# sangyun884/HR-VITON

Measured on AMD Instinct MI355X. Metric: 1024x768 try-on images/sec (train_generator.py step: tocg+glue, G fwd/bwd, D fwd/bwd x2, VGG, Adam), higher is better.
Workload: dtype bf16; 1 GPU; BASELINE configs[3] (SURVEY 8d config #4, headline): train_generator.py 1024x768, 4 img/GPU, --fp16 (bf16 MFMA operands, fp32 accumulate), SPADE ng...; global_batch=4, height=1024, width=768, parallelism=dp1-allreduce, persistent_grid_cus=256, dist_backend=none (single process), world_size=1, rccl_ranks=0

## Files before the change

hr-viton_amd/csrc/conv_f32.hip:

```cpp
#include <stdarg.h>
#include <stdlib.h>
#include <string.h>

#include <vector>

#include "conv_params.h"

namespace hrv {

template <int TM, int TN, int WM, int WN, int VAR, bool BF, int RB = 64>
__device__ __forceinline__ void conv_mfma_tile(const ConvParams& p, const int bid) {
  static_assert(WM * WN == 4 || WM * WN == 8, "4 or 8 MMA waves per block");
  constexpr int NT = 64 * WM * WN;
  constexpr bool SPEC = (VAR & 32) != 0;
  static_assert(RB == 64 || RB == 128, "K-tile row = 64 or 128 bytes");
  constexpr int ES = BF ? 2 : 4;
  constexpr int EPG = 16 / ES;
  constexpr int GPR = RB / 16;
  constexpr int BKE = GPR * EPG;
  constexpr bool GLDS = (VAR & 4) != 0;
  static_assert(!GLDS || (BF && RB == 128), "the LDS-DMA variant exists for the bf16 engine with 128-byte rows");
  constexpr bool SF = (VAR & 8) != 0;
  static_assert(!SF || (BF && !GLDS), "fp32-source variant: bf16 MFMA, register-staged");
  constexpr int LS = GLDS ? RB / 4 : RB / 4 + 4;
  constexpr int BK = RB / 4;
  constexpr int KQ = RB / 32;
  constexpr int RPP = NT / GPR;
  constexpr int BM = 32 * TM * WM;
  constexpr int BN = 32 * TN * WN;
  constexpr int AR = BM / RPP;
  constexpr int BR = (BN * GPR + NT - 1) / NT;
  constexpr bool SWAP = (VAR & 1) != 0;
  constexpr bool PIPE = (VAR & 2) != 0;
  constexpr int ST = (VAR & 16) ? 3 : 2;
  static_assert(ST == 2 || GLDS, "the 3-stage pipeline exists for the LDS-DMA variant");
  static_assert(!SPEC || ST == 3, "wave specialisation rides on the 3-stage LDS-DMA pipeline");
// ... 545 lines not shown
#undef HRV_ADVANCE_ITER
#undef HRV_STORE_TILE
#undef HRV_READ_FRAGS
#undef HRV_MMA1
#undef HRV_MMA_FRAGS

  if (p.splitk > 1) {
    float* wsp = p.ws + (size_t)ks * p.M * p.CoutPad;
#pragma unroll
    for (int j = 0; j < TN; ++j)
#pragma unroll
      for (int i = 0; i < TM; ++i) {
        if (SWAP) {
          const int pidx = row2pix((wm * TM + i) * 32 + l31);
#pragma unroll
          for (int g = 0; g < 4; ++g) {
            const int c0 = n0 + (wn * TN + j) * 32 + 8 * g + 4 * lh;
            if (pidx < p.M) {
              f32x4 v;
#pragma unroll
              for (int e = 0; e < 4; ++e) v[e] = acc[i][j][4 * g + e];
              *reinterpret_cast<f32x4*>(wsp + (size_t)pidx * p.CoutPad + c0) = v;
            }
          }
        } else {
          const int c = n0 + (wn * TN + j) * 32 + l31;
#pragma unroll
          for (int e = 0; e < 16; ++e) {
            const int pidx = row2pix((wm * TM + i) * 32 + 4 * lh + (e & 3) + 8 * (e >> 2));
            if (pidx < p.M) wsp[(size_t)pidx * p.CoutPad + c] = acc[i][j][e];
          }
        }
      }
    return;
  }
  if (!SWAP) {
#pragma unroll
    for (int j = 0; j < TN; ++j) {
      const int c = n0 + (wn * TN + j) * 32 + l31;
      const bool c_ok = c < p.Cout;
      const float sc = (c_ok && p.scale) ? p.scale[c] : 1.f;
      const float sh = (c_ok && p.shift) ? p.shift[c] : 0.f;
#pragma unroll
      for (int i = 0; i < TM; ++i) {
        const int prow0 = (wm * TM + i) * 32 + 4 * lh;
#pragma unroll
        for (int e = 0; e < 16; ++e) {
          const int pidx = row2pix(prow0 + (e & 3) + 8 * (e >> 2));
          if (c_ok && pidx < p.M) {
            float v = acc[i][j][e] * sc + sh;
            const size_t opix = out_pixel(p, pidx);
            if (p.res) v = res_combine(v, ld1rt<BF>(p.res, opix * p.res_cs + p.res_co + c, p.res_f32), p.res_mode, p.slope);
            v = apply_act(v, p.act, p.slope);
            if (!p.out_up) {
              st1rt<BF>(p.out, opix * p.out_cs + p.out_co + c, v, p.out_f32);
            } else {
              const int n = pidx / (p.Ho * p.Wo), rem = pidx - n * (p.Ho * p.Wo);
              const int h = rem / p.Wo, w = rem - h * p.Wo;
              const size_t o = (((size_t)n * 2 * p.Ho + 2 * h) * 2 * p.Wo + 2 * w) * p.out_cs + p.out_co + c;
              st1rt<BF>(p.out, o, v, p.out_f32); st1rt<BF>(p.out, o + p.out_cs, v, p.out_f32);
              st1rt<BF>(p.out, o + (size_t)2 * p.Wo * p.out_cs, v, p.out_f32); st1rt<BF>(p.out, o + (size_t)2 * p.Wo * p.out_cs + p.out_cs, v, p.out_f32);
            }
          }
        }
      }
    }
  } else {
// ... 372 lines not shown

struct TileCfg {
  int TM, TN, WM, WN;
  int RB;
};
static const TileCfg kCfgs[] = {
    {2, 2, 2, 2, 64},
    {1, 3, 4, 1, 64},
    {2, 3, 4, 1, 64},
    {2, 1, 4, 1, 64},
    {2, 2, 4, 1, 64},
    {1, 1, 4, 1, 64},
    {1, 2, 4, 1, 64},
    {4, 2, 2, 2, 64},
    {2, 2, 2, 2, 128},
    {1, 2, 4, 1, 128},
    {4, 2, 2, 2, 128},
    {2, 4, 2, 2, 128},
    {2, 2, 4, 2, 128},
    {2, 2, 4, 2, 128},
    {4, 2, 2, 2, 128},
    {2, 2, 2, 2, 128},
    {2, 2, 4, 2, 128},
    {2, 2, 2, 2, 128},
    {1, 2, 4, 1, 128},
    {2, 2, 4, 1, 128},
};
constexpr int kNumCfgs = sizeof(kCfgs) / sizeof(kCfgs[0]);

static int cfg_bm(int c) { return 32 * kCfgs[c].TM * kCfgs[c].WM; }
static int cfg_bn(int c) { return 32 * kCfgs[c].TN * kCfgs[c].WN; }
static int cfg_rb(int c) { return kCfgs[c].RB; }

static int pick_splitk(int nblk, int KT, bool allowed) {
  if (!allowed || nblk >= 768 || KT < 16) return 1;
  int s = (1024 + nblk - 1) / nblk;
  if (s > 32) s = 32;
  if (s > KT / 8) s = KT / 8;
  return s < 2 ? 1 : s;
}

static int fill_params(const hrv_conv2d_t* d, ConvParams& p, bool need_packed, bool bf = false) {
  const bool srcf = bf && d && ((d->mixed_flags >> 3) & 1);
  const int cm = (bf && !srcf) ? 8 : 4;
  HRV_REQUIRE(d != nullptr, "conv2d: null descriptor");
  const int rb = (need_packed && d->tile_cfg >= 0 && d->tile_cfg < kNumCfgs) ? cfg_rb(d->tile_cfg) : 64;
  HRV_REQUIRE(bf || rb == 64, "conv2d: tile_cfg=%d (128-byte K-tile rows) exists on the bf16 engine only", d->tile_cfg);
  const int bke = rb / (bf ? 2 : 4);
  HRV_REQUIRE(d->nsrc >= 1 && d->nsrc <= HRV_MAX_SRC, "conv2d: nsrc=%d out of range", d->nsrc);
  HRV_REQUIRE(d->N > 0 && d->H > 0 && d->W > 0 && d->Ho > 0 && d->Wo > 0, "conv2d: bad extent");
  HRV_REQUIRE(d->KH > 0 && d->KW > 0 && d->stride > 0 && d->pad >= 0, "conv2d: bad kernel geometry");
  const int padw = d->pad_w_plus1 > 0 ? d->pad_w_plus1 - 1 : d->pad;
  HRV_REQUIRE(d->free_extent ||
                  (d->Ho == (d->H + 2 * d->pad - d->KH) / d->stride + 1 && d->Wo == (d->W + 2 * padw - d->KW) / d->stride + 1),
              "conv2d: Ho/Wo (%d,%d) inconsistent with H,W,k,stride,pad", d->Ho, d->Wo);
  HRV_REQUIRE(d->out_step == 0 || (d->out_step == 2 && d->out_up_shift == 0 && !d->spade && d->out_off_h >= 0 &&
                                   d->out_off_w >= 0 && 2 * (d->Ho - 1) + d->out_off_h < d->out_H &&
                                   2 * (d->Wo - 1) + d->out_off_w < d->out_W),
              "conv2d: out_step/out_off/out_H/out_W inconsistent");
  HRV_REQUIRE(d->res_mode == 0 || d->res_mode == 1, "conv2d: res_mode");
  HRV_REQUIRE(d->Cout > 0 && d->out != nullptr, "conv2d: bad output");
  HRV_REQUIRE((int64_t)d->N * d->Ho * d->Wo < (int64_t)1 << 31, "conv2d: too many output pixels");
  memset(&p, 0, sizeof(p));
  p.bf16 = bf ? 1 : 0;
  p.out_f32 = bf ? (d->mixed_flags & 1) : 1;
  p.res_f32 = bf ? ((d->mixed_flags >> 1) & 1) : 1;
  p.sx_f32 = bf ? ((d->mixed_flags >> 2) & 1) : 1;
  p.src_f32 = srcf ? 1 : 0;
  HRV_REQUIRE(!srcf || rb == 128, "conv2d: fp32-source bf16 mode needs a 128-byte-row tile (cfg 8/9)");
  p.nsrc = d->nsrc;
  int chunks_total = 0;
  bool dma_ok = bf && rb == 128 && !srcf;
// ... 47 lines not shown
  if (d->spade) {
    const hrv_spade_epi_t& e = *d->spade;
    HRV_REQUIRE(need_packed, "conv2d: the SPADE epilogue exists on the MFMA engine only");
    HRV_REQUIRE(e.x && e.mean && e.rstd && d->shift, "conv2d/spade: null pointer");
    HRV_REQUIRE(e.C > 0 && e.C % 4 == 0 && e.x_cstride % 4 == 0 && e.x_coff % 4 == 0 && e.x_coff + e.C <= e.x_cstride,
                "conv2d/spade: channels must be multiples of 4 and in range");
    HRV_REQUIRE(d->Cout == (e.C + 31) / 32 * 64, "conv2d/spade: Cout must be 2*ceil32(C) = %d", (e.C + 31) / 32 * 64);
    HRV_REQUIRE(d->stride == 1 && d->Ho == d->H && d->Wo == d->W, "conv2d/spade: 'same' stride-1 geometry only");
    HRV_REQUIRE((e.noise_z == nullptr) == (e.noise_scale == nullptr), "conv2d/spade: noise_z/noise_scale go together");
    HRV_REQUIRE(d->out_cstride % 4 == 0 && d->out_coff % 4 == 0 && d->out_cstride >= d->out_coff + e.C,
                "conv2d/spade: out slice");
    HRV_REQUIRE((((uintptr_t)e.x | (uintptr_t)e.mean | (uintptr_t)e.rstd | (uintptr_t)e.noise_scale |
                  (uintptr_t)d->shift | (uintptr_t)d->out) & 15) == 0, "conv2d/spade: 16-byte alignment");
    p.epi = 1; p.sx = e.x; p.sx_cs = e.x_cstride; p.sx_co = e.x_coff; p.sC = e.C;
    p.smean = e.mean; p.srstd = e.rstd; p.sz = e.noise_z; p.sns = e.noise_scale; p.sg1p = e.g1p_out;
    p.res = nullptr; p.scale = nullptr;
  } else {
    HRV_REQUIRE(d->out_cstride >= d->out_coff + d->Cout, "conv2d: out slice out of range");
  }
  HRV_REQUIRE(d->residual == nullptr || d->res_cstride >= d->res_coff + d->Cout, "conv2d: residual slice out of range");
  if (need_packed) {
    HRV_REQUIRE(d->tile_cfg >= 0 && d->tile_cfg < kNumCfgs, "conv2d: tile_cfg=%d invalid", d->tile_cfg);
    HRV_REQUIRE(d->w_packed != nullptr && ((uintptr_t)d->w_packed & 15) == 0, "conv2d: w_packed null/unaligned");
    const int bm = cfg_bm(d->tile_cfg), bn = cfg_bn(d->tile_cfg);
    p.wp = (const float*)d->w_packed;
    p.n_tiles = (d->Cout + bn - 1) / bn;
    p.CoutPad = p.n_tiles * bn;
    {
      const int64_t wb = (int64_t)p.KT * p.CoutPad * rb;
      p.w_bytes = (dma_ok && wb < (int64_t)0xFFFFFFF0) ? (unsigned)wb : 0u;
    }
    p.m_tiles = (p.M + bm - 1) / bm;
    p.splitk = 1;
    const char* ev = hrv::env("HRV_CONV_SPLITK");
    int want = pick_splitk(p.m_tiles * p.n_tiles, p.KT, d->spade == nullptr);
    if (ev) want = atoi(ev) > 0 ? atoi(ev) : 1;
    if (d->spade) want = 1;
    if (want > p.KT) want = p.KT;
    if (want > 1) {
      const int64_t need = (int64_t)want * p.M * p.CoutPad * (int64_t)sizeof(float);
      if (d->workspace && d->workspace_bytes >= need && (((uintptr_t)d->workspace) & 15) == 0) {
        p.splitk = want;
        p.ws = (float*)d->workspace;
      }
    }
  } else {
    p.splitk = 1;
  }
  return HRV_OK;
}

constexpr int kDefaultVariant = 1;

template <int TM, int TN, int WM, int WN, int RB = 64>
static int launch_cfg(const ConvParams& p, hipStream_t st) {
  const int nblk = p.m_tiles * p.n_tiles * p.splitk;
  const char* ev = hrv::env("HRV_CONV_VARIANT");
  int var = ev ? atoi(ev) : kDefaultVariant;
  const int oesz = p.out_f32 ? 4 : 2, resz = p.res_f32 ? 4 : 2;
  const bool vec_ok = (p.Cout & 3) == 0 && ((p.out_cs | p.out_co) & 3) == 0 && (!p.res || ((p.res_cs | p.res_co) & 3) == 0) &&
                      (((uintptr_t)p.scale | (uintptr_t)p.shift) & 15) == 0 && (((uintptr_t)p.out) & (4 * oesz - 1)) == 0 &&
                      (((uintptr_t)p.res) & (4 * resz - 1)) == 0;
  if (p.epi == 1) {
    if (TN % 2 != 0) { set_error("conv2d/spade: tile_cfg must have an even TN (cfg 0, 4, 6 or 7)"); return HRV_ERR_ARG; }
    var |= 1;
  } else if (!vec_ok) {
    var &= ~1;
  }
  if (p.bf16) {
    if constexpr (RB == 128 && (32 * TN * WN * 8) % 256 == 0) {
      const char* eg = hrv::env("HRV_CONV_GLDS");
      const bool want = eg ? atoi(eg) != 0 : (32 * TN * WN == 64 || TM * TN >= 8);
      const bool glds = want && p.w_bytes != 0;
      if (p.src_f32) {
        if (var & 1) hipLaunchKernelGGL((conv_mfma_kernel<TM, TN, WM, WN, 9, true, RB>), dim3(nblk), dim3(64 * WM * WN), 0, st, p);
        else hipLaunchKernelGGL((conv_mfma_kernel<TM, TN, WM, WN, 8, true, RB>), dim3(nblk), dim3(64 * WM * WN), 0, st, p);
      } else if (glds) {
        if (var & 1) hipLaunchKernelGGL((conv_mfma_kernel<TM, TN, WM, WN, 5, true, RB>), dim3(nblk), dim3(64 * WM * WN), 0, st, p);
        else hipLaunchKernelGGL((conv_mfma_kernel<TM, TN, WM, WN, 4, true, RB>), dim3(nblk), dim3(64 * WM * WN), 0, st, p);
      } else {
        if (var & 1) hipLaunchKernelGGL((conv_mfma_kernel<TM, TN, WM, WN, 1, true, RB>), dim3(nblk), dim3(64 * WM * WN), 0, st, p);
        else hipLaunchKernelGGL((conv_mfma_kernel<TM, TN, WM, WN, 0, true, RB>), dim3(nblk), dim3(64 * WM * WN), 0, st, p);
      }
    } else {
      if (var & 1) hipLaunchKernelGGL((conv_mfma_kernel<TM, TN, WM, WN, 1, true, RB>), dim3(nblk), dim3(64 * WM * WN), 0, st, p);
      else hipLaunchKernelGGL((conv_mfma_kernel<TM, TN, WM, WN, 0, true, RB>), dim3(nblk), dim3(64 * WM * WN), 0, st, p);
    }
  } else if constexpr (RB != 64) {
    set_error("conv2d: 128-byte K-tile rows exist on the bf16 engine only");
    return HRV_ERR_ARG;
  } else {
    switch (var) {
      case 0: hipLaunchKernelGGL((conv_mfma_kernel<TM, TN, WM, WN, 0, false>), dim3(nblk), dim3(64 * WM * WN), 0, st, p); break;
      case 1: hipLaunchKernelGGL((conv_mfma_kernel<TM, TN, WM, WN, 1, false>), dim3(nblk), dim3(64 * WM * WN), 0, st, p); break;
      case 2: hipLaunchKernelGGL((conv_mfma_kernel<TM, TN, WM, WN, 2, false>), dim3(nblk), dim3(64 * WM * WN), 0, st, p); break;
      case 3: hipLaunchKernelGGL((conv_mfma_kernel<TM, TN, WM, WN, 3, false>), dim3(nblk), dim3(64 * WM * WN), 0, st, p); break;
      default: set_error("conv2d: HRV_CONV_VARIANT=%d invalid", var); return HRV_ERR_ARG;
    }
  }
  int rc = check_launch("conv_mfma_kernel");
  if (rc || p.splitk <= 1) return rc;
  const size_t total = (size_t)p.M * ((p.Cout + 3) / 4);
  const size_t gsz = (total + 255) / 256;
  const dim3 g((unsigned)(gsz > 4096 ? 4096 : gsz));
  if (p.bf16) hipLaunchKernelGGL(splitk_reduce_kernel<true>, g, dim3(256), 0, st, p);
  else hipLaunchKernelGGL(splitk_reduce_kernel<false>, g, dim3(256), 0, st, p);
  return check_launch("splitk_reduce_kernel");
}

template <int TM, int TN, int WM, int WN, bool ST3, bool SPECW = false>
static int launch_cfg8w(const ConvParams& p, hipStream_t st) {
  const int nblk = p.m_tiles * p.n_tiles * p.splitk;
  const int oesz = p.out_f32 ? 4 : 2, resz = p.res_f32 ? 4 : 2;
  const bool vec_ok = (p.Cout & 3) == 0 && ((p.out_cs | p.out_co) & 3) == 0 && (!p.res || ((p.res_cs | p.res_co) & 3) == 0) &&
                      (((uintptr_t)p.scale | (uintptr_t)p.shift) & 15) == 0 && (((uintptr_t)p.out) & (4 * oesz - 1)) == 0 &&
                      (((uintptr_t)p.res) & (4 * resz - 1)) == 0;
  if (!p.bf16 || p.src_f32 || p.w_bytes == 0) {
    set_error("conv2d: tile_cfg 12/13 (eight-wave LDS-DMA) needs bf16-stored sources within the 32-bit buffer range");
    return HRV_ERR_ARG;
  }
  constexpr int V = 4 | (ST3 ? 16 : 0) | (SPECW ? 32 : 0);
  constexpr int NTB = 64 * WM * WN * (SPECW ? 2 : 1);
  if (vec_ok || p.epi == 1)
    hipLaunchKernelGGL((conv_mfma_kernel<TM, TN, WM, WN, V | 1, true, 128>), dim3(nblk), dim3(NTB), 0, st, p);
  else
    hipLaunchKernelGGL((conv_mfma_kernel<TM, TN, WM, WN, V, true, 128>), dim3(nblk), dim3(NTB), 0, st, p);
  int rc = check_launch("conv_mfma_kernel");
  if (rc || p.splitk <= 1) return rc;
  const size_t total = (size_t)p.M * ((p.Cout + 3) / 4);
  const size_t gsz = (total + 255) / 256;
  const dim3 g((unsigned)(gsz > 4096 ? 4096 : gsz));
  hipLaunchKernelGGL(splitk_reduce_kernel<true>, g, dim3(256), 0, st, p);
  return check_launch("splitk_reduce_kernel");
}

static bool patch_eligible(const ConvParams& p) {
  return p.bf16 && !p.src_f32 && p.nsrc == 1 && p.KH == 3 && p.KW == 3 && p.stride == 1 && p.pad == 1 && p.pad_w == 1 &&
         p.Ho == p.H && p.Wo == p.W && p.src[0].up_shift == 0 && p.src[0].C % 128 == 0 && p.src[0].bytes != 0 &&
         p.w_bytes != 0 && p.out_step != 2;
}

template <int TMP, int TNP, int WMP, int WNP, int STV>
static int launch_patch(const ConvParams& p0, hipStream_t st, int n0_base = 0, int n_cols_tiles = 0) {
  constexpr int BNP = 32 * TNP * WNP;
  if (!patch_eligible(p0) || (n_cols_tiles == 0 && p0.CoutPad % BNP != 0) || n0_base + n_cols_tiles * BNP > p0.CoutPad) {
    set_error("conv2d: tile_cfg 16-18 (patch mode) needs a 3x3 stride-1 'same' convolution over one bf16-stored source with "
              "C %% 128 == 0");
    return HRV_ERR_ARG;
  }
  ConvParams p = p0;
  p.splitk = 1;
  constexpr int THP = TMP * WMP * 32 / 16;
  p.m_tiles = p.N * ((p.H + THP - 1) / THP) * ((p.W + 15) / 16);
  p.n_tiles = n_cols_tiles > 0 ? n_cols_tiles : p.CoutPad / BNP;
  p.n0_base = n0_base;
  const int nblk = p.m_tiles * p.n_tiles;
  const int oesz = p.out_f32 ? 4 : 2, resz = p.res_f32 ? 4 : 2;
  const bool vec_ok = (p.Cout & 3) == 0 && ((p.out_cs | p.out_co) & 3) == 0 && (!p.res || ((p.res_cs | p.res_co) & 3) == 0) &&
                      (((uintptr_t)p.scale | (uintptr_t)p.shift) & 15) == 0 && (((uintptr_t)p.out) & (4 * oesz - 1)) == 0 &&
                      (((uintptr_t)p.res) & (4 * resz - 1)) == 0;
  constexpr int V = 4 | STV | 64;
  const int n_cu = persistent_cus();
  p.tlog = diag_tlog(p.m_tiles);
  constexpr int PATCH_LDS = ((TMP * WMP * 32 / 16 + 2) * 18 * 64 + ((STV & 16) ? 3 : 2) * BNP * 32) * 4;
  const int per_cu = PATCH_LDS <= 80 * 1024 ? 2 : 1;
  const char* ep = hrv::env("HRV_PATCH_PERSIST");
  int grid = (ep && ep[0] == '0') ? nblk : n_cu * per_cu;
  if (grid > nblk) grid = nblk;
  if (vec_ok || p.epi == 1)
    hipLaunchKernelGGL((conv_mfma_kernel<TMP, TNP, WMP, WNP, V | 1, true, 128>), dim3(grid), dim3(64 * WMP * WNP), 0, st, p);
  else
    hipLaunchKernelGGL((conv_mfma_kernel<TMP, TNP, WMP, WNP, V, true, 128>), dim3(grid), dim3(64 * WMP * WNP), 0, st, p);
  return check_launch("conv_mfma_kernel[patch]");
}

static int launch_any(int tile_cfg, const ConvParams& p, hipStream_t st) {
  switch (tile_cfg) {
    case 0: return launch_cfg<2, 2, 2, 2>(p, st);
    case 1: return launch_cfg<1, 3, 4, 1>(p, st);
    case 2: return launch_cfg<2, 3, 4, 1>(p, st);
    case 3: return launch_cfg<2, 1, 4, 1>(p, st);
    case 4: return launch_cfg<2, 2, 4, 1>(p, st);
    case 5: return launch_cfg<1, 1, 4, 1>(p, st);
    case 6: return launch_cfg<1, 2, 4, 1>(p, st);
    case 7: return launch_cfg<4, 2, 2, 2>(p, st);
    case 8: return launch_cfg<2, 2, 2, 2, 128>(p, st);
    case 9: return launch_cfg<1, 2, 4, 1, 128>(p, st);
    case 10: return launch_cfg<4, 2, 2, 2, 128>(p, st);
    case 11: return launch_cfg<2, 4, 2, 2, 128>(p, st);
    case 12: return launch_cfg8w<2, 2, 4, 2, false>(p, st);
    case 13: return launch_cfg8w<2, 2, 4, 2, true>(p, st);
    case 14: return launch_cfg8w<4, 2, 2, 2, true, true>(p, st);
    case 15: return launch_cfg8w<2, 2, 2, 2, true, true>(p, st);
    case 16: return launch_patch<2, 2, 4, 2, 16>(p, st);
    case 17: return launch_patch<2, 2, 2, 2, 0>(p, st);
    case 18: {
      const char* e3 = hrv::env("HRV_CONV_PATCH_ST3");
      if (e3 && e3[0] == '0') return launch_patch<1, 2, 4, 1, 0>(p, st);
      const char* es = hrv::env("HRV_CONV_PATCH_SPLIT");
      const int c64 = p.CoutPad / 64;
      if (c64 >= 3 && !(es && es[0] == '0')) {
        const int rc = launch_patch<2, 2, 2, 2, 0>(p, st, 0, c64 / 2);
        if (rc) return rc;
        return launch_patch<1, 2, 4, 1, 16>(p, st, (c64 / 2) * 128, c64 - 2 * (c64 / 2));
      }
      return launch_patch<1, 2, 4, 1, 16>(p, st);
    }
    case 19: return launch_patchw(p, st);
  }
  set_error("conv2d: tile_cfg=%d invalid", tile_cfg);
  return HRV_ERR_ARG;
}

}

using namespace hrv;

extern "C" int hrv_conv2d_tile_bn(int32_t c) { return (c >= 0 && c < kNumCfgs) ? cfg_bn(c) : -1; }
extern "C" int hrv_conv2d_tile_bm(int32_t c) { return (c >= 0 && c < kNumCfgs) ? cfg_bm(c) : -1; }
extern "C" int hrv_conv2d_tile_row_bytes(int32_t c) { return (c >= 0 && c < kNumCfgs) ? cfg_rb(c) : -1; }
// ... 33 lines not shown
  HRV_REQUIRE(tile_cfg >= 0 && tile_cfg < kNumCfgs && cfg_rb(tile_cfg) == 64, "pack_weight: bad tile_cfg %d", tile_cfg);
  HRV_REQUIRE(nsrc >= 1 && nsrc <= HRV_MAX_SRC, "pack_weight: bad nsrc");
  constexpr int BK = HOST_BK;
  const int bn = cfg_bn(tile_cfg);
  const int64_t cpad = (int64_t)((Cout + bn - 1) / bn) * bn;
  int cin_real = 0, chunks_total = 0;
  for (int i = 0; i < nsrc; ++i) {
    HRV_REQUIRE(srcC_real[i] > 0 && srcC_real[i] <= srcC[i] && srcC[i] % 4 == 0, "pack_weight: bad channel counts");
    cin_real += srcC_real[i];
    chunks_total += (srcC[i] + BK - 1) / BK;
  }
  const int64_t total = (int64_t)KH * KW * chunks_total * cpad * BK;
  memset(out, 0, sizeof(float) * total);
  for (int kh = 0; kh < KH; ++kh)
    for (int kw = 0; kw < KW; ++kw) {
      int chunk0 = 0, cbase = 0;
      for (int s = 0; s < nsrc; ++s) {
        const int chunks = (srcC[s] + BK - 1) / BK;
        for (int c = 0; c < srcC_real[s]; ++c) {
          const int64_t kt = (int64_t)(kh * KW + kw) * chunks_total + chunk0 + c / BK;
          float* dst = out + (kt * cpad) * BK + (c % BK);
          const float* srcw = w + ((int64_t)(cbase + c) * KH + kh) * KW + kw;
          const int64_t ostride = (int64_t)cin_real * KH * KW;
          for (int co = 0; co < Cout; ++co) dst[(int64_t)co * BK] = srcw[co * ostride];
        }
        chunk0 += chunks;
        cbase += srcC_real[s];
      }
    }
  return HRV_OK;
}

extern "C" int64_t hrv_conv2d_workspace_bytes(const hrv_conv2d_t* d) {
  if (!d || d->tile_cfg < 0 || d->tile_cfg >= kNumCfgs || d->spade) return 0;
  const int bm = cfg_bm(d->tile_cfg), bn = cfg_bn(d->tile_cfg);
  const int64_t M = (int64_t)d->N * d->Ho * d->Wo;
  const int n_tiles = (d->Cout + bn - 1) / bn;
  const int m_tiles = (int)((M + bm - 1) / bm);
  int chunks = 0;
  for (int i = 0; i < d->nsrc && i < HRV_MAX_SRC; ++i) chunks += (d->src[i].C + HOST_BK - 1) / HOST_BK;
  const int KT = d->KH * d->KW * chunks;
  const char* ev = hrv::env("HRV_CONV_SPLITK");
  int s = pick_splitk(m_tiles * n_tiles, KT, true);
  if (ev) s = atoi(ev) > 0 ? atoi(ev) : 1;
  if (s > KT) s = KT;
  return s > 1 ? (int64_t)s * M * n_tiles * bn * (int64_t)sizeof(float) : 0;
}

static int conv2d_one(const hrv_conv2d_t* d, hipStream_t stream, bool bf) {
  ConvParams p;
  int rc = fill_params(d, p, true, bf);
  if (rc) return rc;
  return launch_any(d->tile_cfg, p, stream);
}

static int conv2d_any(const hrv_conv2d_t* d, hipStream_t stream, bool bf) {
  HRV_REQUIRE(d != nullptr, "conv2d: null descriptor");
  HRV_REQUIRE(d->nsrc >= 1 && d->nsrc <= HRV_MAX_SRC && d->N > 0 && d->H > 0 && d->W > 0, "conv2d: bad geometry");
  int64_t per_img = 0;
  for (int i = 0; i < d->nsrc; ++i) {
    const hrv_src_t& s = d->src[i];
    const int sr = s.up_shift > 0 ? s.up_shift : 0, sl = s.up_shift < 0 ? -s.up_shift : 0;
    const int64_t e = (int64_t)((d->H >> sr) << sl) * ((d->W >> sr) << sl) * s.cstride;
    per_img = e > per_img ? e : per_img;
  }
  const int64_t out_px = (int64_t)d->Ho * d->Wo;
  const bool srcf0 = bf && (d->mixed_flags & 8);
  const int64_t lim = (int64_t)0xFFFFFFF0 / ((bf && !srcf0) ? 2 : 4);
  int64_t cap = d->N;
  if (const char* e = hrv::env("HRV_CONV_MAX_BATCH")) {
    const long long v = atoll(e);
    if (v > 0 && v < cap) cap = v;
  }
  const bool fits = cap == d->N && d->N * per_img < lim && d->N * out_px < ((int64_t)1 << 31);
  const bool plain_fwd = d->out_step <= 1 && d->free_extent == 0 && d->res_mode == 0;
  if (fits || !plain_fwd || per_img <= 0 || out_px <= 0) return conv2d_one(d, stream, bf);
  int64_t nb = (lim - 1) / per_img;
  const int64_t nb2 = (((int64_t)1 << 31) - 1) / out_px;
  nb = nb < nb2 ? nb : nb2;
// ... 118 lines not shown
```

hr-viton_amd/csrc/conv_params.h:

```cpp
#pragma once
#include "hrv_common.h"

namespace hrv {

typedef float f32x16 __attribute__((ext_vector_type(16)));
typedef float f32x4 __attribute__((ext_vector_type(4)));

constexpr int HOST_BK = 16;

struct SrcDev {
  const float* ptr;
  int C, cstride, coff, up_shift, pre_act, chunks;
  unsigned bytes;
};

struct ConvParams {
  SrcDev src[HRV_MAX_SRC];
  int nsrc;
  int N, H, W, Ho, Wo, KH, KW, stride, pad;
  int M;
  int Cout, CoutPad;
  int chunks_total;
  int KT;
  int m_tiles, n_tiles;
  int n0_base;
  const float* wp;
  const float* scale;
  const float* shift;
  const float* res;
  int res_cs, res_co;
  int act;
  float slope;
  float pre_slope;
  float* out;
  int out_cs, out_co;
  int splitk;
  float* ws;
  int pad_w;
  int out_up;
  int out_step, out_oh, out_ow, out_H, out_W;
  int bf16;
  int out_f32, res_f32, sx_f32;
  int src_f32;
  int res_mode;
  unsigned w_bytes;
  int epi;
  const float* sx;
  int sx_cs, sx_co, sC;
  const float* smean;
  const float* srstd;
  const float* sz;
  const float* sns;
  float* sg1p;
  unsigned long long* tlog;
};

__device__ __forceinline__ size_t out_pixel(const ConvParams& p, int pidx) {
  if (p.out_step != 2) return (size_t)pidx;
  const int n = pidx / (p.Ho * p.Wo), rem = pidx - n * (p.Ho * p.Wo);
  const int h = rem / p.Wo, w = rem - h * p.Wo;
  return ((size_t)n * p.out_H + 2 * h + p.out_oh) * p.out_W + 2 * w + p.out_ow;
}

__device__ __forceinline__ float res_combine(float v, float r, int mode, float slope) {
  return mode == 0 ? v + r : v * (r > 0.f ? 1.f : slope);
}

typedef __bf16 bf16x8 __attribute__((ext_vector_type(8)));
typedef unsigned short u16x4 __attribute__((ext_vector_type(4)));

// ... 92 lines not shown
```

hr-viton_amd/ops.py:

```python
from __future__ import annotations

import ctypes as C
import os
from dataclasses import dataclass
from typing import Optional, Sequence, Tuple, Union

import weakref

import torch

from . import _lib
from ._lib import ACT_LRELU, ACT_NONE, ACT_RELU, ACT_TANH, HrvError


WEIGHTS_EPOCH = [0]
LOAD_EPOCH = [0]


def weights_epoch(tensors) -> int:
    return sum(getattr(t, "_hrv_epoch", 0) for t in tensors)


def _ceil4(c: int) -> int:
    return (c + 3) // 4 * 4
# ... 148 lines not shown
    _Prof.enabled = False
    torch.cuda.synchronize()
    out = [((k, n, fl, by, s.elapsed_time(e), kn) if kernels else (k, n, fl, by, s.elapsed_time(e)))
           for (k, n, fl, by, kn, s, e) in _Prof.records]
    _Prof.records = []
    return out


class _Timed:
    def __init__(self, kind, name, flops, nbytes, kernel=None):
        self.args = (kind, name, flops, nbytes, kernel or kind)

    def __enter__(self):
        if _Prof.enabled:
            self.s = torch.cuda.Event(enable_timing=True)
            self.e = torch.cuda.Event(enable_timing=True)
            self.s.record()
        return self

    def __exit__(self, *a):
        if _Prof.enabled:
            self.e.record()
            _Prof.records.append((*self.args, self.s, self.e))
        return False


_WS = {}
GRAPH_WATCH = weakref.WeakSet()


WS_PER_STREAM = [False]


def _workspace(device, nbytes: int) -> torch.Tensor:
    key = (str(device), torch.cuda.current_stream(device).cuda_stream if WS_PER_STREAM[0] else 0)
    t = _WS.get(key)
    if t is None or t.numel() * 4 < nbytes:
        t = torch.empty((nbytes + 3) // 4, dtype=torch.float32, device=device)
        _WS[key] = t
    return t


SrcSpec = Union[Act, Tuple[Act, int, int]]


class ConvLayer:

    def __init__(self, weight: torch.Tensor, src_real: Sequence[int], device, scale: Optional[torch.Tensor] = None,
                 shift: Optional[torch.Tensor] = None, stride: int = 1, pad: int = 1, act: int = ACT_NONE,
                 slope: float = 0.2, name: str = "conv", bf16: bool = False, out_f32: bool = False,
                 mma_bf16: bool = False):
        assert not (bf16 and mma_bf16)
        self.bf16 = bf16
        self.mixed = mma_bf16
        self.out_f32 = out_f32 or not bf16
        w = weight.detach().to("cpu", torch.float32).contiguous()
        self.Cout, cin, self.KH, self.KW = w.shape
        assert sum(src_real) == cin, (name, src_real, cin)
        assert 1 <= len(src_real) <= _lib.HRV_MAX_SRC
        self.w_cpu = w
        self.src_real = list(src_real)
        self.src_pad = [_cpad(c, bf16) for c in src_real]
        self.device = device
        self.stride, self.pad, self.act, self.slope, self.name = stride, pad, act, slope, name
        self.scale = None if scale is None else scale.detach().to(device, torch.float32).contiguous()
        self.shift = None if shift is None else shift.detach().to(device, torch.float32).contiguous()
        self._packed = {}
        self._w_dev = None

    def _get_packed(self, cfg: int) -> torch.Tensor:
        if cfg not in self._packed:
            lib = _lib.load()
            n = len(self.src_pad)
# ... 53 lines not shown
            cfg = lib.hrv_conv2d_pick_tile(N * Ho * Wo, self.Cout)
            if self.mixed:
                cfg = 8 if (self.Cout + 127) // 128 * 128 <= (self.Cout + 63) // 64 * 64 else 9
            if self.bf16 and cfg in (0, 6):
                cfg = 8 if cfg == 0 else 9
            if self.bf16 and self.KH == 1 and self.KW == 1 and sum(self.src_pad) <= 128 and self.Cout % 64 == 0:
                cfg = 6
            pt = patch_tile(self.bf16, self.KH, self.KW, self.stride, self.pad, len(specs), up0, self.src_pad[0],
                            self.Cout, N, H, W)
            cfg = pt or cfg
        forced = os.environ.get("HRV_CONV_TILE") if (spade is None and not self.mixed) else None
        if forced is not None:
            cfg = int(forced)
        d.Cout, d.tile_cfg = self.Cout, cfg
        if naive:
            if self._w_dev is None:
                self._w_dev = self.w_cpu.to(self.device)
            d.w_oihw = self._w_dev.data_ptr()
        else:
            d.w_packed = self._get_packed(cfg).data_ptr()
        d.scale = None if self.scale is None else self.scale.data_ptr()
        d.shift = None if self.shift is None else self.shift.data_ptr()
        if residual is not None:
            assert (residual.N, residual.H, residual.W) == (N, Ho, Wo) and residual.C == self.Cout
            d.residual, d.res_cstride, d.res_coff = residual.t.data_ptr(), residual.cstride, residual.coff
        d.act, d.act_slope = self.act, self.slope
        assert (out.N, out.H, out.W) == (N, Ho << out_up, Wo << out_up) and out.C == oc, (self.name, out.t.shape, out.C)
        d.out, d.out_cstride, d.out_coff = out.t.data_ptr(), out.cstride, out.coff
        d.out_up_shift = out_up
        if spade is not None:
            d.spade = C.pointer(spade)
            mixed |= 4 if getattr(spade, "_x_f32", True) else 0
        d.mixed_flags = 15 if self.mixed else (mixed if self.bf16 else 0)
        if not naive and spade is None:
            need = lib.hrv_conv2d_workspace_bytes(C.byref(d))
            if need > 0:
                ws = _workspace(a0.t.device, need)
                d.workspace, d.workspace_bytes = ws.data_ptr(), ws.numel() * 4
        engine_bf16 = self.bf16 or self.mixed
        fn = lib.hrv_conv2d_naive_nhwc_f32 if naive else (lib.hrv_conv2d_nhwc_bf16 if engine_bf16 else lib.hrv_conv2d_nhwc_f32)
        assert not (naive and engine_bf16), "the naive cross-check is fp32"
        nbytes = (sum(act_bytes(a) for a, _, _ in specs) + act_bytes(out) + act_bytes(residual) +
                  self.Cout * sum(self.src_real) * self.KH * self.KW * (2 if engine_bf16 else 4))
        if spade is not None:
            nbytes += N * Ho * Wo * oc * (4 if getattr(spade, "_x_f32", True) else 2)
        with _Timed("conv", self.name, self.flops(N, Ho, Wo), nbytes, f"conv_mfma_kernel[tile {d.tile_cfg}]"):
            _lib.check(fn(C.byref(d), _stream()), f"hrv_conv2d_nhwc_f32[{self.name}]")
        return out


class TapConvLayer:

    def __init__(self, weight: torch.Tensor, src_real: Sequence[int], device, bias: Optional[torch.Tensor] = None,
                 name: str = "tapconv", mma_bf16: bool = False):
        w = weight.detach().to("cpu", torch.float32)
        self.Cout, cin, self.KH, self.KW = w.shape
        assert self.KH == self.KW and self.KH % 2 == 1
        self.pad = self.KH // 2
        w1 = w.permute(2, 3, 0, 1).reshape(self.KH * self.KW * self.Cout, cin, 1, 1).contiguous()
        self.inner = ConvLayer(w1, src_real, device, stride=1, pad=0, name=name + "[taps-as-channels 1x1]",
                               mma_bf16=mma_bf16)
        self.bias = None if bias is None else bias.detach().to(device, torch.float32).contiguous()
        self.name = name

    def __call__(self, srcs, out: Act, residual: Optional[Act] = None) -> Act:
        lib = _lib.load()
        y = self.inner(srcs)
        res_ptr, rcs = (None, 0) if residual is None else (residual.t.data_ptr(), residual.cstride)
        if residual is not None:
            assert residual.coff == 0 and residual.C == self.Cout
# ... 204 lines not shown
```

hr-viton_amd/train_ops.py:

```python
from __future__ import annotations

import ctypes as C
import itertools
import os
from typing import Optional, Sequence, Tuple

import torch

from . import _lib, ops
from .ops import ACT_LRELU, ACT_NONE, ACT_RELU, Act, _ceil4, _stream, _Timed, _workspace


MMA_BF16 = [False]


def _bf16_tile(cout: int) -> int:
    p64, p128 = (cout + 63) // 64 * 64, (cout + 127) // 128 * 128
    return 8 if p128 <= p64 else 9


_FROZEN_PACKS: dict = {}


def evict_serving_packs(tokens):
    toks = set(tokens)
    dead = [k for k in _FROZEN_PACKS
            if any(isinstance(e, tuple) and len(e) == 3 and e[0] == "serve" and e[1] in toks for e in k)]
    for k in dead:
        del _FROZEN_PACKS[k]
    return len(dead)


class _Side:
    streams: dict = {}
    pending: dict = {}
    active = [False]


def wgrad_side_maxpix() -> int:
    if os.environ.get("HRV_WGRAD_SIDE", "0") != "1":
        return 0
    return int(os.environ.get("HRV_WGRAD_SIDE_MAXPIX", "65536") or 0)

# ... 300 lines not shown
    bp = (C.c_void_p * n)(*[g.data_ptr() for g in gbs])
    _lib.check(lib.hrv_shared_taps_grad_f32(dw.data_ptr(), db.data_ptr(), n, hid, c, cp, gp, bp, _stream()),
               "hrv_shared_taps_grad_f32")


def _run_engine(srcs, w_packed, Cout, cfg, N, H, W, Ho, Wo, KH, KW, stride, pad_h, pad_w, out: Act, scale=None,
                shift=None, residual: Optional[Act] = None, res_mode: int = 0, act: int = ACT_NONE, slope: float = 0.2,
                free_extent: int = 0, out_step: int = 0, out_off=(0, 0), out_hw=(0, 0), out_up: int = 0,
                name: str = "conv", flops: float = 0.0, mma_bf16: bool = False, spade=None):
    lib = _lib.load()
    d = _lib.hrv_conv2d_t()
    d.N, d.H, d.W, d.Ho, d.Wo = N, H, W, Ho, Wo
    d.KH, d.KW, d.stride, d.pad = KH, KW, stride, pad_h
    d.pad_w_plus1 = pad_w + 1
    d.nsrc = len(srcs)
    src_bf16 = srcs[0][0].bf16
    for i, (a, up, creal) in enumerate(srcs):
        s = d.src[i]
        assert a.bf16 == src_bf16, f"{name}: the sources of one convolution share one storage type"
        s.ptr, s.C, s.cstride, s.coff, s.up_shift, s.pre_act, s.C_real = (a.t.data_ptr(), ops._cpad(creal, a.bf16),
                                                                          a.cstride, a.coff, up, 0, creal)
    d.w_packed = w_packed.data_ptr()
    d.Cout, d.tile_cfg = Cout, cfg
    d.scale = None if scale is None else scale.data_ptr()
    d.shift = None if shift is None else shift.data_ptr()
    if residual is not None:
        d.residual, d.res_cstride, d.res_coff = residual.t.data_ptr(), residual.cstride, residual.coff
    d.res_mode = res_mode
    d.act, d.act_slope = act, slope
    d.out, d.out_cstride, d.out_coff = out.t.data_ptr(), out.cstride, out.coff
    d.out_up_shift = out_up
    d.free_extent, d.out_step = free_extent, out_step
    d.out_off_h, d.out_off_w, d.out_H, d.out_W = out_off[0], out_off[1], out_hw[0], out_hw[1]
    need = lib.hrv_conv2d_workspace_bytes(C.byref(d))
    if need > 0:
        ws = _workspace(out.t.device, need)
        d.workspace, d.workspace_bytes = ws.data_ptr(), ws.numel() * 4
    if spade is not None:
        d.spade = C.pointer(spade)
    if mma_bf16:
        d.mixed_flags = ((0 if out.bf16 else 1) | (0 if (residual is not None and residual.bf16) else 2) | 4 |
                         (0 if src_bf16 else 8))
    else:
        assert not (src_bf16 or out.bf16 or (residual is not None and residual.bf16)), f"{name}: bf16 tensors need MMA_BF16"
    nbytes = (sum(ops.act_bytes(a, creal) for a, _, creal in srcs) + ops.act_bytes(out, Cout) +
             
              ops.act_bytes(residual, Cout) + float(Cout) * sum(c for _, _, c in srcs) * KH * KW * (2 if mma_bf16 else 4))
    with _Timed("conv", name, flops, nbytes, f"conv_mfma_kernel[tile {cfg}]"):
        fn = lib.hrv_conv2d_nhwc_bf16 if mma_bf16 else lib.hrv_conv2d_nhwc_f32
        _lib.check(fn(C.byref(d), _stream()), f"hrv_conv2d_nhwc_{'bf16' if mma_bf16 else 'f32'}[{name}]")
    return out


def _thin_ok(a: Act, KH: int, KW: int, stride: int, pad: int, cols: int, N: int, H: int, W: int) -> bool:
    import os
    return (MMA_BF16[0] and a.bf16 and stride == 1 and KH == KW and pad == KH // 2 and N * H * W >= 65536 and
            os.environ.get("HRV_THIN_CONV", "1") != "0" and
            bool(_lib.load().hrv_thin_conv_supported(KH, KW, a.Cp, cols)))


def _thin_conv(src: Act, w: torch.Tensor, mode: int, sigma, wscale: float, shift, residual: Optional[Act], res_mode: int,
               act: int, slope: float, out: Act, name: str, flops: float):
    lib = _lib.load()
    d = _lib.hrv_thin_conv_t()
    d.src, d.N, d.H, d.W = src.t.data_ptr(), src.N, src.H, src.W
    d.src_channels, d.src_cstride, d.src_coff = src.Cp, src.cstride, src.coff
    d.w_oihw, d.Cout, d.Cin, d.KH, d.KW = w.data_ptr(), w.shape[0], w.shape[1], w.shape[2], w.shape[3]
    d.sigma = None if sigma is None else sigma.data_ptr()
    d.wscale, d.mode = wscale, mode
    d.shift = None if shift is None else shift.data_ptr()
    if residual is not None:
        d.residual, d.res_cstride, d.res_coff = residual.t.data_ptr(), residual.cstride, residual.coff
# ... 1015 lines not shown
```

Before: 61.39 images/s.

## Reduce split-K partials in-launch via last-arriving block with atomic tile counters

Split-K convolutions now finish inside the main kernel. Each block writes its partial slab, bumps a per-tile atomic counter in the workspace head, and the last-arriving block sums all slabs and runs the normal fused epilogue. This removes the separate reduction kernel launch. It also allows split-K for SPADE convolutions, adds smaller-M tile variants for small problems, and caps per-tile slab bytes. The cost is extra fences and atomics, plus a serialized reduction done by one block, and the workspace counters must stay zeroed across calls.

```diff
diff --git a/hr-viton_amd/csrc/conv_f32.hip b/hr-viton_amd/csrc/conv_f32.hip
--- a/hr-viton_amd/csrc/conv_f32.hip
+++ b/hr-viton_amd/csrc/conv_f32.hip
@@ -2,6 +2,7 @@
 #include <stdlib.h>
 #include <string.h>
 
+#include <type_traits>
 #include <vector>
 
 #include "conv_params.h"
@@ -613,7 +614,73 @@
           }
         }
       }
-    return;
+    if (SPEC || PATCH || p.tile_cnt == nullptr) return;
+    asm volatile("s_waitcnt vmcnt(0)" ::: "memory");
+    __syncthreads();
+    int* last_flag = reinterpret_cast<int*>(smem);
+    if (tid == 0) {
+      __builtin_amdgcn_fence(__ATOMIC_RELEASE, "agent");
+      asm volatile("s_waitcnt vmcnt(0)" ::: "memory");
+      const unsigned ticket = __hip_atomic_fetch_add(p.tile_cnt + lid, 1u, __ATOMIC_RELAXED, __HIP_MEMORY_SCOPE_AGENT);
+      const int last = ticket == (unsigned)(p.splitk - 1);
+      if (last) {
+        __builtin_amdgcn_fence(__ATOMIC_ACQUIRE, "agent");
+        asm volatile("s_waitcnt vmcnt(0)" ::: "memory");
+        __hip_atomic_store(p.tile_cnt + lid, 0u, __ATOMIC_RELAXED, __HIP_MEMORY_SCOPE_AGENT);
+      }
+      *last_flag = last;
+    }
+    __syncthreads();
+    if (!*last_flag) return;
+#pragma unroll
+    for (int i = 0; i < TM; ++i)
+#pragma unroll
+      for (int j = 0; j < TN; ++j)
+#pragma unroll
+        for (int e = 0; e < 16; ++e) acc[i][j][e] = 0.f;
+    constexpr int RU = TM * TN <= 2 ? 4 : 2;
+    auto add_slabs = [&](const int s0, auto ns_c) {
+      constexpr int NS = decltype(ns_c)::value;
+      f32x16 t[NS][TM][TN];
+#pragma unroll
+      for (int u = 0; u < NS; ++u) {
+        const float* src = p.ws + (size_t)(s0 + u) * p.M * p.CoutPad;
+#pragma unroll
+        for (int j = 0; j < TN; ++j)
+#pragma unroll
+          for (int i = 0; i < TM; ++i) {
+            if (SWAP) {
+              const int pidx = min(row2pix((wm * TM + i) * 32 + l31), p.M - 1);
+#pragma unroll
+              for (int g = 0; g < 4; ++g) {
+                const int c0 = n0 + (wn * TN + j) * 32 + 8 * g + 4 * lh;
+                const f32x4 v = *reinterpret_cast<const f32x4*>(src + (size_t)pidx * p.CoutPad + c0);
+#pragma unroll
+                for (int e = 0; e < 4; ++e) t[u][i][j][4 * g + e] = v[e];
+              }
+            } else {
+              const int c = n0 + (wn * TN + j) * 32 + l31;
+#pragma unroll
+              for (int e = 0; e < 16; ++e) {
+                const int pidx = min(row2pix((wm * TM + i) * 32 + 4 * lh + (e & 3) + 8 * (e >> 2)), p.M - 1);
+                t[u][i][j][e] = src[(size_t)pidx * p.CoutPad + c];
+              }
+            }
+          }
+      }
+#pragma unroll
+      for (int u = 0; u < NS; ++u) {
+#pragma unroll
+        for (int i = 0; i < TM; ++i)
+#pragma unroll
+          for (int j = 0; j < TN; ++j)
+#pragma unroll
+            for (int e = 0; e < 16; ++e) acc[i][j][e] += t[u][i][j][e];
+      }
+    };
+    int s0 = 0;
+    for (; s0 + RU <= p.splitk; s0 += RU) add_slabs(s0, std::integral_constant<int, RU>{});
+    for (; s0 < p.splitk; ++s0) add_slabs(s0, std::integral_constant<int, 1>{});
   }
   if (!SWAP) {
 #pragma unroll
@@ -1052,12 +1119,51 @@
 static int cfg_bn(int c) { return 32 * kCfgs[c].TN * kCfgs[c].WN; }
 static int cfg_rb(int c) { return kCfgs[c].RB; }
 
+constexpr int kSplitkCounters = 4096;
+constexpr int64_t kSplitkCounterBytes = kSplitkCounters * 4;
+
 static int pick_splitk(int nblk, int KT, bool allowed) {
   if (!allowed || nblk >= 768 || KT < 16) return 1;
   int s = (1024 + nblk - 1) / nblk;
   if (s > 32) s = 32;
   if (s > KT / 8) s = KT / 8;
   return s < 2 ? 1 : s;
+}
+
+static bool inlaunch_on() {
+  const char* e = hrv::env("HRV_SPLITK_INLAUNCH");
+  return !(e && e[0] == '0');
+}
+static bool inlaunch_cfg(int c) { return c >= 0 && c <= 13; }
+static bool small_m_cfg(int c, bool spade) { return c == 8 || (c == 9 && !spade); }
+
+struct SplitPlan {
+  int bm_small, m_tiles, splitk;
+};
+static SplitPlan plan_split(int cfg, int64_t M, int n_tiles, int KT, bool spade, bool inl) {
+  const int bm = cfg_bm(cfg), bn = cfg_bn(cfg);
+  SplitPlan sp;
+  sp.bm_small = 0;
+  sp.m_tiles = (int)((M + bm - 1) / bm);
+  if (!inl) {
+    sp.splitk = spade ? 1 : pick_splitk(sp.m_tiles * n_tiles, KT, true);
+    return sp;
+  }
+  if (M <= 1024 && small_m_cfg(cfg, spade)) {
+    sp.bm_small = 1;
+    sp.m_tiles = (int)((M + 63) / 64);
+  }
+  const int tiles = sp.m_tiles * n_tiles;
+  const int64_t tile_bytes = (int64_t)(sp.bm_small ? 64 : bm) * bn * 4;
+  int s = 1;
+  if (tiles < 768 && KT >= 16 && tiles <= kSplitkCounters) {
+    s = (512 + tiles - 1) / tiles;
+    if (s < 2) s = 2;
+    if (s > KT / 8) s = KT / 8;
+    while (s > 2 && s * tile_bytes > 256 * 1024) --s;
+  }
+  sp.splitk = s < 2 ? 1 : s;
+  return sp;
 }
 
 static int fill_params(const hrv_conv2d_t* d, ConvParams& p, bool need_packed, bool bf = false) {
@@ -1171,16 +1277,26 @@
     }
     p.m_tiles = (p.M + bm - 1) / bm;
     p.splitk = 1;
+    const bool inl = inlaunch_on() && inlaunch_cfg(d->tile_cfg);
+    const SplitPlan sp = plan_split(d->tile_cfg, p.M, p.n_tiles, p.KT, d->spade != nullptr, inl);
     const char* ev = hrv::env("HRV_CONV_SPLITK");
-    int want = pick_splitk(p.m_tiles * p.n_tiles, p.KT, d->spade == nullptr);
+    int want = sp.splitk;
     if (ev) want = atoi(ev) > 0 ? atoi(ev) : 1;
-    if (d->spade) want = 1;
+    if (d->spade && !inl) want = 1;
     if (want > p.KT) want = p.KT;
     if (want > 1) {
-      const int64_t need = (int64_t)want * p.M * p.CoutPad * (int64_t)sizeof(float);
-      if (d->workspace && d->workspace_bytes >= need && (((uintptr_t)d->workspace) & 15) == 0) {
+      const int m_tiles = inl ? sp.m_tiles : p.m_tiles;
+      const int64_t head = inl ? kSplitkCounterBytes : 0;
+      const int64_t need = head + (int64_t)want * p.M * p.CoutPad * (int64_t)sizeof(float);
+      if (d->workspace && d->workspace_bytes >= need && (((uintptr_t)d->workspace) & 15) == 0 &&
+          (!inl || m_tiles * p.n_tiles <= kSplitkCounters)) {
         p.splitk = want;
-        p.ws = (float*)d->workspace;
+        p.ws = (float*)((char*)d->workspace + head);
+        if (inl) {
+          p.tile_cnt = (unsigned*)d->workspace;
+          p.bm_small = sp.bm_small;
+          p.m_tiles = m_tiles;
+        }
       }
     }
   } else {
@@ -1238,7 +1354,7 @@
     }
   }
   int rc = check_launch("conv_mfma_kernel");
-  if (rc || p.splitk <= 1) return rc;
+  if (rc || p.splitk <= 1 || p.tile_cnt) return rc;
   const size_t total = (size_t)p.M * ((p.Cout + 3) / 4);
   const size_t gsz = (total + 255) / 256;
   const dim3 g((unsigned)(gsz > 4096 ? 4096 : gsz));
@@ -1265,7 +1381,7 @@
   else
     hipLaunchKernelGGL((conv_mfma_kernel<TM, TN, WM, WN, V, true, 128>), dim3(nblk), dim3(NTB), 0, st, p);
   int rc = check_launch("conv_mfma_kernel");
-  if (rc || p.splitk <= 1) return rc;
+  if (rc || p.splitk <= 1 || p.tile_cnt) return rc;
   const size_t total = (size_t)p.M * ((p.Cout + 3) / 4);
   const size_t gsz = (total + 255) / 256;
   const dim3 g((unsigned)(gsz > 4096 ? 4096 : gsz));
@@ -1323,8 +1439,8 @@
     case 5: return launch_cfg<1, 1, 4, 1>(p, st);
     case 6: return launch_cfg<1, 2, 4, 1>(p, st);
     case 7: return launch_cfg<4, 2, 2, 2>(p, st);
-    case 8: return launch_cfg<2, 2, 2, 2, 128>(p, st);
-    case 9: return launch_cfg<1, 2, 4, 1, 128>(p, st);
+    case 8: return p.bm_small ? launch_cfg<1, 2, 2, 2, 128>(p, st) : launch_cfg<2, 2, 2, 2, 128>(p, st);
+    case 9: return p.bm_small ? launch_cfg<1, 1, 2, 2, 128>(p, st) : launch_cfg<1, 2, 4, 1, 128>(p, st);
     case 10: return launch_cfg<4, 2, 2, 2, 128>(p, st);
     case 11: return launch_cfg<2, 4, 2, 2, 128>(p, st);
     case 12: return launch_cfg8w<2, 2, 4, 2, false>(p, st);
@@ -1424,19 +1540,20 @@
 }
 
 extern "C" int64_t hrv_conv2d_workspace_bytes(const hrv_conv2d_t* d) {
-  if (!d || d->tile_cfg < 0 || d->tile_cfg >= kNumCfgs || d->spade) return 0;
-  const int bm = cfg_bm(d->tile_cfg), bn = cfg_bn(d->tile_cfg);
+  if (!d || d->tile_cfg < 0 || d->tile_cfg >= kNumCfgs) return 0;
+  const bool inl = inlaunch_on() && inlaunch_cfg(d->tile_cfg);
+  if (d->spade && !inl) return 0;
+  const int bn = cfg_bn(d->tile_cfg);
   const int64_t M = (int64_t)d->N * d->Ho * d->Wo;
   const int n_tiles = (d->Cout + bn - 1) / bn;
-  const int m_tiles = (int)((M + bm - 1) / bm);
   int chunks = 0;
   for (int i = 0; i < d->nsrc && i < HRV_MAX_SRC; ++i) chunks += (d->src[i].C + HOST_BK - 1) / HOST_BK;
   const int KT = d->KH * d->KW * chunks;
   const char* ev = hrv::env("HRV_CONV_SPLITK");
-  int s = pick_splitk(m_tiles * n_tiles, KT, true);
+  int s = plan_split(d->tile_cfg, M, n_tiles, KT, d->spade != nullptr, inl).splitk;
   if (ev) s = atoi(ev) > 0 ? atoi(ev) : 1;
   if (s > KT) s = KT;
-  return s > 1 ? (int64_t)s * M * n_tiles * bn * (int64_t)sizeof(float) : 0;
+  return s > 1 ? (inl ? kSplitkCounterBytes : 0) + (int64_t)s * M * n_tiles * bn * (int64_t)sizeof(float) : 0;
 }
 
 static int conv2d_one(const hrv_conv2d_t* d, hipStream_t stream, bool bf) {
diff --git a/hr-viton_amd/csrc/conv_params.h b/hr-viton_amd/csrc/conv_params.h
--- a/hr-viton_amd/csrc/conv_params.h
+++ b/hr-viton_amd/csrc/conv_params.h
@@ -36,6 +36,8 @@
   int out_cs, out_co;
   int splitk;
   float* ws;
+  int bm_small;
+  unsigned* tile_cnt;
   int pad_w;
   int out_up;
   int out_step, out_oh, out_ow, out_H, out_W;
diff --git a/hr-viton_amd/ops.py b/hr-viton_amd/ops.py
--- a/hr-viton_amd/ops.py
+++ b/hr-viton_amd/ops.py
@@ -204,13 +204,25 @@
 WS_PER_STREAM = [False]
 
 
-def _workspace(device, nbytes: int) -> torch.Tensor:
+WS_HEAD_BYTES = 16384
+
+
+def _ws_tensor(device, nbytes: int) -> torch.Tensor:
     key = (str(device), torch.cuda.current_stream(device).cuda_stream if WS_PER_STREAM[0] else 0)
     t = _WS.get(key)
     if t is None or t.numel() * 4 < nbytes:
-        t = torch.empty((nbytes + 3) // 4, dtype=torch.float32, device=device)
+        t = torch.empty((max(nbytes, WS_HEAD_BYTES) + 3) // 4, dtype=torch.float32, device=device)
+        t[:WS_HEAD_BYTES // 4].zero_()
         _WS[key] = t
     return t
+
+
+def _workspace(device, nbytes: int) -> torch.Tensor:
+    return _ws_tensor(device, WS_HEAD_BYTES + nbytes)[WS_HEAD_BYTES // 4:]
+
+
+def _conv_workspace(device, nbytes: int) -> torch.Tensor:
+    return _ws_tensor(device, nbytes)
 
 
 SrcSpec = Union[Act, Tuple[Act, int, int]]
@@ -330,10 +342,10 @@
             d.spade = C.pointer(spade)
             mixed |= 4 if getattr(spade, "_x_f32", True) else 0
         d.mixed_flags = 15 if self.mixed else (mixed if self.bf16 else 0)
-        if not naive and spade is None:
+        if not naive:
             need = lib.hrv_conv2d_workspace_bytes(C.byref(d))
             if need > 0:
-                ws = _workspace(a0.t.device, need)
+                ws = _conv_workspace(a0.t.device, need)
                 d.workspace, d.workspace_bytes = ws.data_ptr(), ws.numel() * 4
         engine_bf16 = self.bf16 or self.mixed
         fn = lib.hrv_conv2d_naive_nhwc_f32 if naive else (lib.hrv_conv2d_nhwc_bf16 if engine_bf16 else lib.hrv_conv2d_nhwc_f32)
diff --git a/hr-viton_amd/train_ops.py b/hr-viton_amd/train_ops.py
--- a/hr-viton_amd/train_ops.py
+++ b/hr-viton_amd/train_ops.py
@@ -8,7 +8,7 @@
 import torch
 
 from . import _lib, ops
-from .ops import ACT_LRELU, ACT_NONE, ACT_RELU, Act, _ceil4, _stream, _Timed, _workspace
+from .ops import ACT_LRELU, ACT_NONE, ACT_RELU, Act, _ceil4, _conv_workspace, _stream, _Timed, _workspace
 
 
 MMA_BF16 = [False]
@@ -375,12 +375,12 @@
     d.out_up_shift = out_up
     d.free_extent, d.out_step = free_extent, out_step
     d.out_off_h, d.out_off_w, d.out_H, d.out_W = out_off[0], out_off[1], out_hw[0], out_hw[1]
+    if spade is not None:
+        d.spade = C.pointer(spade)
     need = lib.hrv_conv2d_workspace_bytes(C.byref(d))
     if need > 0:
-        ws = _workspace(out.t.device, need)
+        ws = _conv_workspace(out.t.device, need)
         d.workspace, d.workspace_bytes = ws.data_ptr(), ws.numel() * 4
-    if spade is not None:
-        d.spade = C.pointer(spade)
     if mma_bf16:
         d.mixed_flags = ((0 if out.bf16 else 1) | (0 if (residual is not None and residual.bf16) else 2) | 4 |
                          (0 if src_bf16 else 8))
```

Result: slower. 57.89 images/s, median of 2 (-5.7%).
